# AIS-Bonn/lattice_net

Hardware: AMD Instinct MI355X
Metric: Mpoints/sec splat+conv+slice fwd+bwd on 120k-pt SemanticKITTI scan (higher is better)
Workload: dtype f32 (convolution products bf16x3-emulated)

## Files before the change

### include/latticenet_hip.h

```cpp
#ifndef LATTICENET_HIP_H
#define LATTICENET_HIP_H

#include <stddef.h>

#ifdef __cplusplus
extern "C" {
#endif

#define LN_OK 0
#define LN_ERR_ARG (-1)
#define LN_ERR_UNSUPPORTED (-2)
#define LN_ERR_LAUNCH (-3)
#define LN_ERR_WORKSPACE (-4)

#define LN_STATUS_TABLE_FULL 1
#define LN_STATUS_KEY_RANGE 2
#define LN_STATUS_BUCKET_OVERFLOW 4

#define LN_MAX_POS_DIM 6
#define LN_SLOT_MAP_INTS 32
#define LN_KEYS_RAW 0
#define LN_KEYS_LATTICE 1
#define LN_NOT_VISITED (-2)

// ... 44 lines not shown

int ln_table_bucket_count(int capacity);
int ln_build_concurrency(int scans_in_flight);

size_t ln_build_workspace_bytes(long long tokens, int capacity);

#define LN_BUILD_WRITE_IDX 1
#define LN_BUILD_CLEAR_FIRST 2
#define LN_BUILD_ATOMIC_PATH 4
#define LN_BUILD_CANONICAL_ROWS 8
#define LN_BUILD_SORTED_CSR 16
int ln_build_splat(const LnTable* t, const float* positions_raw, const float* sigmas_host, int n, int* idx, float* w,
                   int flags, const LnCsr* csr, void* workspace, size_t workspace_bytes, float* clear_values,
                   long long clear_values_elems, void* stream);

int ln_canonicalize(const LnTable* t, int* idx, long long tokens, const LnCsr* csr, void* workspace, size_t workspace_bytes, void* stream);

int ln_rehash(const LnTable* t, void* stream);

int ln_splat_accumulate(float* table_values, const float* vals, const int* idx, const float* w, int n, int pos_dim,
                        int val_dim, void* stream);

long long ln_csr_max_segments(long long tokens, int groups_upper);
size_t ln_csr_workspace_bytes(long long tokens, int groups_upper);
int ln_csr_build(const int* idx, long long tokens, int groups_upper, const LnCsr* csr, void* workspace, size_t workspace_bytes,
                 void* stream);
int ln_csr_reduce_rows(const LnCsr* csr, const int* grp_row, long long max_segments, const float* src, const float* w, int val_dim,
                       int src_div, int src_stride, float* dst, void* stream);
int ln_csr_sort(const LnCsr* csr, int groups_upper, void* workspace, size_t workspace_bytes, long long tokens, void* stream);

// ... 144 lines not shown
```

### lattice_net_amd/_lib.py

```python
from __future__ import annotations

import ctypes as C
import os

import torch

_PKG = os.path.dirname(os.path.abspath(__file__))
LIB_PATH = os.environ.get("LATTICE_NET_LIB") or os.path.join(_PKG, "liblatticenet_hip.so")

LN_STATUS_TABLE_FULL = 1
LN_STATUS_KEY_RANGE = 2
LN_STATUS_BUCKET_OVERFLOW = 4
LN_BUILD_WRITE_IDX = 1
LN_BUILD_CLEAR_FIRST = 2
LN_BUILD_ATOMIC_PATH = 4
LN_BUILD_CANONICAL_ROWS = 8
LN_BUILD_SORTED_CSR = 16
LN_NOT_VISITED = -2
LN_CONV_FLIP_NEIGHBOURS = 1
LN_CONV_TRANSPOSED_FILTER = 2
LN_CONV_BANK_READY = 4
LN_MAX_POS_DIM = 6
LN_KEYS_RAW = 0
LN_KEYS_LATTICE = 1
LN_XCD_GROUPS = 8
LN_SLOT_MAP_INTS = 32


class LnTable(C.Structure):

    _fields_ = [
        ("capacity", C.c_int),
# ... 39 lines not shown
_CSR = C.POINTER(LnCsr)

SIGNATURES = {
    "ln_last_error_string": (C.c_char_p, []),
    "ln_version": (C.c_char_p, []),
    "ln_abi_hash": (C.c_char_p, []),
    "ln_kernel_names": (C.c_char_p, []),
    "ln_profile_begin": (_i, [C.c_char_p, _i]),
    "ln_profile_end": (_i, [C.POINTER(C.c_double), C.POINTER(_i)]),
    "ln_profile_end_table": (_i, [C.c_char_p, _i]),
    "ln_table_clear": (_i, [_T, _vp, _ll, _vp]),
    "ln_build_workspace_bytes": (_sz, [_ll, _i]),
    "ln_table_bucket_count": (_i, [_i]),
    "ln_build_concurrency": (_i, [_i]),
    "ln_build_splat": (_i, [_T, _vp, _vp, _i, _vp, _vp, _i, _CSR, _vp, _sz, _vp, _ll, _vp]),
    "ln_rehash": (_i, [_T, _vp]),
    "ln_canonicalize": (_i, [_T, _vp, _ll, _CSR, _vp, _sz, _vp]),
    "ln_splat_accumulate": (_i, [_vp, _vp, _vp, _vp, _i, _i, _i, _vp]),
    "ln_csr_workspace_bytes": (_sz, [_ll, _i]),
    "ln_csr_max_segments": (_ll, [_ll, _i]),
    "ln_csr_build": (_i, [_vp, _ll, _i, _CSR, _vp, _sz, _vp]),
    "ln_csr_reduce_rows": (_i, [_CSR, _vp, _ll, _vp, _vp, _i, _i, _i, _vp, _vp]),
    "ln_csr_sort": (_i, [_CSR, _i, _vp, _sz, _ll, _vp]),
    "ln_splat_accumulate_and_neighbours": (_i, [_CSR, _vp, _ll, _vp, _vp, _i, _i, _i, _vp, _T, _i, _vp, _vp]),
    "ln_csr_segment_max": (_i, [_CSR, _vp, _ll, _vp, _i, _i, _vp, _vp, _vp, _vp]),
    "ln_csr_group_sizes": (_i, [_CSR, _vp, _i, _i, _vp, _vp]),
    "ln_distribute": (_i, [_T, _vp, _vp, _vp, _i, _i, _vp, _vp, _vp, _i, _CSR, _vp, _sz, _vp, _ll, _vp]),
    "ln_coarsen": (_i, [_T, _i, _T, _CSR, _vp, _sz, _vp]),
    "ln_neighbours": (_i, [_T, _i, _T, _i, _i, _i, _i, _vp, _vp]),
    "ln_im2row": (_i, [_vp, _vp, _i, _i, _i, _vp, _vp]),
# ... 108 lines not shown
```

### lattice_net_amd/csrc/ln_table.hip

```cpp
#include "ln_common.h"
#include "ln_simplex.h"
#include "ln_csr.h"
#include "ln_neighbours.h"

#include <stdarg.h>
#include <stdio.h>
#include <string.h>

static thread_local char g_ln_error[512] = "";

void ln_set_error(const char* fmt, ...) {
    va_list ap;
    va_start(ap, fmt);
    vsnprintf(g_ln_error, sizeof(g_ln_error), fmt, ap);
    va_end(ap);
}

int ln_check_launch(const char* what) {
    hipError_t e = hipGetLastError();
    if (e != hipSuccess) {
        ln_set_error("%s: %s", what, hipGetErrorString(e));
        return LN_ERR_LAUNCH;
    }
    return LN_OK;
}

extern "C" const char* ln_last_error_string(void) { return g_ln_error; }

#include <vector>
namespace {
struct LnProfState {
    char names[256] = "";
    int max_samples = 0;
    std::vector<hipEvent_t> starts, stops;
    std::vector<const char*> sample_names;
    size_t used = 0;
    long long dropped = 0;
};
LnProfState g_prof;
}

LnProfEvents ln_prof_next(const char* name) {
    LnProfEvents ev{nullptr, nullptr, false};
// ... 283 lines not shown
        for (int i = 0; i < D; ++i) o[i] = pr[i] / sc.sigma[i];
        for (int j = 0; j < val_dim; ++j) o[D + j] = vals[(size_t)p * val_dim + j];
        o[D + val_dim] = b;
    }
}


#ifndef LN_KEYS_PTS_SMALL_D
#define LN_KEYS_PTS_SMALL_D 2
#endif
#define LN_KEYS_PTS_PER_THREAD ((D) <= 3 ? LN_KEYS_PTS_SMALL_D : 1)
#define LN_KEYS_PTS_PER_BLOCK (256 * LN_KEYS_PTS_PER_THREAD)
template <int D, int TH>
__global__ void __launch_bounds__(TH)
    k_point_keys(LnTable t, const float* __restrict__ pos_raw, LnScale<D> sc, int n, int sb, int nbk, int capb,
                 int* __restrict__ part_tok, unsigned long long* __restrict__ part_pk, int* __restrict__ tok_slot,
                 float* __restrict__ w, const float* __restrict__ vals, int val_dim, float* __restrict__ distributed,
                 int* __restrict__ seg_count, int seg_regions, float* __restrict__ clear_values, long long clear_values_elems,
                 unsigned int* __restrict__ pub) {
    constexpr bool SPLIT = TH == 1024;
    constexpr int PTS = TH == 256 ? LN_KEYS_PTS_PER_THREAD : 1;
    constexpr int RH = SPLIT ? (D + 2) / 2 : D + 1;
    constexpr int PTS_PER_BLOCK = SPLIT ? 512 : TH * PTS;
    __shared__ int s_cnt[LN_BKT_MAX];
    __shared__ int s_lbase[LN_BKT_MAX];
    __shared__ int s_scan_tmp[TH / 64];
    __shared__ unsigned long long s_stage_pk[PTS_PER_BLOCK * (D + 1)];
    __shared__ int s_stage_tok[PTS_PER_BLOCK * (D + 1)];
    __shared__ int s_stage_dst[PTS_PER_BLOCK * (D + 1)];
    int* cursor = t.slot_cnt;
    LN_STAMP(0);
    for (int b = threadIdx.x; b < nbk; b += TH) s_cnt[b] = 0;
    const LnSlotMap smap = ln_load_slot_map(t.slot_map);
    ln_lds_barrier();
    LN_STAMP(1);
    unsigned long long pk[PTS][RH];
    int bkt[PTS][RH];
    int rank[PTS][RH];
    bool bad_key = false;
    const int r_first = SPLIT ? (threadIdx.x & 1) * RH : 0;
#pragma unroll
    for (int it = 0; it < PTS; ++it) {
        const int p = SPLIT ? blockIdx.x * PTS_PER_BLOCK + (threadIdx.x >> 1) : blockIdx.x * PTS_PER_BLOCK + it * TH + threadIdx.x;
#pragma unroll
        for (int k = 0; k < RH; ++k) bkt[it][k] = -1;
        if (p >= n) continue;
        float pr[D];
#pragma unroll
        for (int i = 0; i < D; ++i) pr[i] = pos_raw[(size_t)p * D + i];
        LnSimplex<D> s;
        ln_simplex<D>(pr, sc, s);
        ln_simplex_of_cloud<D>(s, p, t.batch_points, t.batch_key_step);
#pragma unroll
        for (int k = 0; k < RH; ++k) {
            const int r = r_first + k;
            if (SPLIT && r > D) continue;
            int key[D];
            ln_vertex_key<D>(s, r, key);
            float bary = s.bary[0];
#pragma unroll
            for (int q = 1; q <= D; ++q) bary = (r == q) ? s.bary[q] : bary;
            const size_t tk = (size_t)p * (D + 1) + r;
            const bool lat_fmt = t.key_format == LN_KEYS_LATTICE;
            const bool ok = lat_fmt ? KeyPack<D>::lattice_in_range(key, r) : KeyPack<D>::in_range(key, t.key_format);
            if (ok) {
                pk[it][k] = lat_fmt ? KeyPack<D>::lattice_pack(key, r) : KeyPack<D>::pack(key, t.key_format);
                bkt[it][k] = LnProbe::bucket_of_key<D>(key, t.capacity, sb, smap);
                rank[it][k] = atomicAdd(&s_cnt[bkt[it][k]], 1);
            } else {
                bad_key = true;
                if (tok_slot) tok_slot[tk] = -1;
            }
            if (w) w[tk] = ok ? bary : -1.0f;
            if (distributed) {
                const int row_len = D + val_dim + 1;
                float* o = distributed + tk * row_len;
#pragma unroll
// ... 22 lines not shown
    }
    LN_STAMP(4);
    ln_lds_barrier();
    LN_STAMP(5);
#pragma unroll
    for (int it = 0; it < PTS; ++it) {
        const int p = SPLIT ? blockIdx.x * PTS_PER_BLOCK + (threadIdx.x >> 1) : blockIdx.x * PTS_PER_BLOCK + it * TH + threadIdx.x;
#pragma unroll
        for (int k = 0; k < RH; ++k) {
            if (bkt[it][k] < 0) continue;
            const int tk = p * (D + 1) + r_first + k;
            const int at = s_cnt[bkt[it][k]] + rank[it][k];
            const int j = s_lbase[bkt[it][k]] + rank[it][k];
            s_stage_tok[j] = tk;
            s_stage_pk[j] = pk[it][k];
            s_stage_dst[j] = at < capb ? bkt[it][k] * capb + at : -1;
        }
    }
    ln_lds_barrier();
    LN_STAMP(6);
    for (int j = threadIdx.x; j < block_tokens; j += TH) {
        const int dst = s_stage_dst[j];
        const int tk = s_stage_tok[j];
        if (dst >= 0) {
            part_tok[dst] = tk;
            part_pk[dst] = s_stage_pk[j];
        } else if (tok_slot) {
            tok_slot[tk] = -1;
        }
    }
    {
        const long long stride = (long long)gridDim.x * TH;
        const long long g = (long long)blockIdx.x * TH + threadIdx.x;
        if (clear_values) {
            const long long n4 = clear_values_elems >> 2;
            float4* v4 = reinterpret_cast<float4*>(clear_values);
            for (long long i = g; i < n4; i += stride) v4[i] = make_float4(0.f, 0.f, 0.f, 0.f);
            for (long long i = (n4 << 2) + g; i < clear_values_elems; i += stride) clear_values[i] = 0.f;
        }
        const long long nk = (long long)t.capacity * D;
        for (long long i = g; i < nk; i += stride) t.keys[i] = 0;
// ... 12 lines not shown
#ifndef LN_BKT_THREADS
#define LN_BKT_THREADS 1024
#endif
#define LN_BKT_WAVES (LN_BKT_THREADS / 64)
#ifndef LN_BKT_NARROW_TOKENS
#define LN_BKT_NARROW_TOKENS 4096
#endif
static thread_local int g_ln_build_concurrency = 1;
extern "C" int ln_build_concurrency(int scans_in_flight) {
    g_ln_build_concurrency = scans_in_flight > 1 ? scans_in_flight : 1;
    return LN_OK;
}
#define LN_BKT_LDS_LIMIT (150 * 1024)
#define LN_BKT_LDS_PER_SLOT (sizeof(unsigned long long) + 7 * sizeof(int))
#define LN_BKT_LDS_EXTRA 32
#ifndef LN_BKT_REG_TOK
#define LN_BKT_REG_TOK 4
#endif
#define LN_PUB_READY 0x80000000u
#define LN_PUB_ERR 0x40000000u
#define LN_PUB_CNT 0x3FFFFFFFu
template <int D, int TH>
__global__ void __launch_bounds__(TH)
    k_bucket_rows(LnTable t, int sb, int nbk, int capb, int* __restrict__ cursor, const int* __restrict__ part_tok,
                  const unsigned long long* __restrict__ part_pk, int* __restrict__ part_slot, int* __restrict__ part_pos,
                  int* __restrict__ idx_out, LnCsr csr, unsigned int* __restrict__ pub) {
    extern __shared__ __attribute__((aligned(16))) unsigned long long s_mem[];
    unsigned long long* skeys = s_mem;
    int* scnt = reinterpret_cast<int*>(skeys + sb);
    unsigned int* smin = reinterpret_cast<unsigned int*>(scnt + sb);
    int* soff = reinterpret_cast<int*>(smin + sb);
    int* sseg = soff + sb;
    int* srow = sseg + sb;
    int* srank = srow + sb;
    unsigned int* slist = reinterpret_cast<unsigned int*>(s_mem) + ((8 * sb + 3) & ~3);
    __shared__ int s_wave_tok[16], s_wave_seg[16], s_wave_new[16];
    __shared__ int s_run_tok, s_run_seg, s_run_new, s_err;
    __shared__ int s_rcnt[LN_XCD_GROUPS], s_rbase[LN_XCD_GROUPS];
    __shared__ int s_ticket;
    const int tid = threadIdx.x;
    const int lane = tid & 63;
    const int wave = tid >> 6;
    if (tid == 0) s_ticket = atomicAdd(reinterpret_cast<int*>(&pub[nbk]), 1);
    LN_STAMP(8);
    for (int i = tid; i < sb; i += TH) {
        skeys[i] = LN_EMPTY_KEY;
        scnt[i] = 0;
        smin[i] = LN_EMPTY_TOK;
    }
    ln_lds_barrier();
    const int b = s_ticket;
    const bool mapped = t.slot_map != nullptr;
    const LnBucket bk(b, t.capacity, sb, t.slot_map);
    const int lo = bk.lo;
    const int size = bk.size;
    const size_t in0 = (size_t)b * capb;
    int before = 0;
    for (int i = tid; i < b; i += TH) before += min(cursor[i], capb);
    const int my_cursor = cursor[b];
    const int ntok = min(my_cursor, capb);
    int r_tk[LN_BKT_REG_TOK], r_ls[LN_BKT_REG_TOK], r_pos[LN_BKT_REG_TOK];
    unsigned long long r_pk[LN_BKT_REG_TOK];
#pragma unroll
    for (int k = 0; k < LN_BKT_REG_TOK; ++k) {
        const int j = tid + k * TH;
        r_ls[k] = -1;
        r_pos[k] = -1;
        r_tk[k] = j < ntok ? part_tok[in0 + j] : -1;
        r_pk[k] = j < ntok ? part_pk[in0 + j] : LN_EMPTY_KEY;
    }
#pragma unroll
    for (int off = 32; off >= 1; off >>= 1) before += __shfl_xor(before, off, 64);
    if (lane == 0) s_wave_tok[wave] = before;
    if (tid == 0) {
        s_run_tok = 0;
        s_run_seg = 0;
        s_run_new = 0;
        s_err = my_cursor > capb ? 1 : 0;
    }
    if (tid < LN_XCD_GROUPS) s_rcnt[tid] = 0;
    __syncthreads();
    int base = 0;
#pragma unroll
    for (int k = 0; k < (TH / 64); ++k) base += s_wave_tok[k];
// ... 191 lines not shown
    const int new_here = s_run_new;
    if (t.row_regions && tid == 0 && slot_ordered) {
        const int bpr = nbk / LN_XCD_GROUPS;
        if (b % bpr == 0) t.row_regions[b / bpr] = base_row;
        if (b == nbk - 1) t.row_regions[LN_XCD_GROUPS] = base_row + new_here;
    }
    LN_STAMP(12);
    for (int i = tid; i < size; i += TH) {
        const int h = lo + i;
        const int beg = base + soff[i];
        const int c = scnt[i];
        int row = -1;
        if (c) {
            row = base_row + srow[i];
            if (t.row_limit > 0 && row >= t.row_limit) row = -1;
        }
        srow[i] = row;
        csr.grp_start[h] = beg;
        const unsigned long long pk = skeys[i];
        t.slot_keys[h] = pk;
        t.entries[h] = row;
        t.slot_tok[h] = smin[i];
        if (row >= 0) {
            int key[D];
            KeyPack<D>::unpack(pk, key, t.key_format);
#pragma unroll
            for (int k = 0; k < D; ++k) t.keys[(size_t)row * D + k] = key[k];
        }
        const int sr = planes ? (sseg[i] >> 28) : bucket_region;
        long long sid = (long long)sr * csr.seg_region + s_rbase[planes ? sr : 0] + (planes ? (sseg[i] & 0x0FFFFFFF) : sseg[i]);
// ... 8 lines not shown
            t.slot_tok[h] = LN_EMPTY_TOK;
        }
        if (tid == 0) {
            csr.grp_start[t.capacity] = base + ntok;
            const int total = base_row + new_here;
            int bits = (err_all ? LN_STATUS_BUCKET_OVERFLOW : 0) | (cursor[nbk] ? LN_STATUS_KEY_RANGE : 0);
            *t.nr_filled = total;
            if (bits) atomicOr(t.status, bits);
            ln_report_to_host(t.host_counters, total, bits, t.host_seq);
        }
        __syncthreads();
        for (int i = tid; i <= nbk; i += TH) cursor[i] = 0;
    }
    ln_lds_barrier();
    LN_STAMP(13);
#pragma unroll
    for (int k = 0; k < LN_BKT_REG_TOK; ++k) {
        if (r_tk[k] < 0) continue;
        if (r_ls[k] >= 0) csr.csr_tok[base + soff[r_ls[k]] + r_pos[k]] = r_tk[k];
        if (idx_out) idx_out[r_tk[k]] = r_ls[k] >= 0 ? srow[r_ls[k]] : -1;
    }
    for (int j = tid + LN_BKT_REG_TOK * TH; j < ntok; j += TH) {
        const int ls = part_slot[in0 + j];
        const int tk = part_tok[in0 + j];
        if (ls >= 0) csr.csr_tok[base + soff[ls] + part_pos[in0 + j]] = tk;
        if (idx_out) idx_out[tk] = ls >= 0 ? srow[ls] : -1;
    }
    for (int j = placed + tid; j < ntok; j += TH)
        csr.csr_tok[base + j] = -1;
    LN_STAMP(14);
}

template <int D>
__global__ void __launch_bounds__(256)
    k_insert_coarse(LnTable fine, int fine_rows_upper, LnTable coarse, int* __restrict__ tok_slot, int* __restrict__ tok_pos) {
    constexpr int TPR = 2 * (D + 1) + 1;
    const int r = blockIdx.x * blockDim.x + threadIdx.x;
    int m = *fine.nr_filled;
    if (m > fine_rows_upper) m = fine_rows_upper;
    if (r >= fine_rows_upper) return;
    int* ts = tok_slot + (size_t)r * TPR;
    int* tp = tok_pos + (size_t)r * TPR;
    for (int j = 0; j < TPR; ++j) {
        ts[j] = -1;
        tp[j] = -1;
// ... 168 lines not shown

struct BuildWs {
    unsigned long long* bitmap;
    int* block_cnt;
    int* block_prefix;
    int* tok_slot;
    int* tok_pos;
    void* csr_ws;
    size_t csr_ws_bytes;
    int nb;
    int capb;
    unsigned long long* part_pk;
    int* part_tok;
    int* part_slot;
    int* part_pos;
    unsigned int* pub;
};

static size_t ln_align256(size_t x) { return (x + 255) & ~size_t(255); }

static int ln_bucket_region(long long tokens, int capacity) {
    const int nbk = ln_bucket_count(capacity);
    long long capb = 16 * ((tokens + nbk - 1) / nbk) + 1024;
    capb = (capb + 63) & ~63ll;
    return int(capb);
}

extern "C" int ln_table_bucket_count(int capacity) { return capacity > 0 ? ln_bucket_count(capacity) : 0; }

extern "C" size_t ln_build_workspace_bytes(long long tokens, int capacity) {
    if (tokens < 1) tokens = 1;
    if (capacity < 1) capacity = 1;
    const size_t nb = (size_t)ln_div_up(tokens, 256);
    const size_t region = (size_t)ln_bucket_count(capacity) * ln_bucket_region(tokens, capacity);
    return ln_align256(nb * 4 * sizeof(unsigned long long)) + 2 * ln_align256(nb * sizeof(int)) +
           2 * ln_align256((size_t)tokens * sizeof(int)) + ln_align256(ln_csr_scan_workspace_bytes(capacity)) +
           ln_align256(region * sizeof(unsigned long long)) + 3 * ln_align256(region * sizeof(int)) +
           ln_align256(((size_t)ln_bucket_count(capacity) + 1) * sizeof(unsigned int));
}

static int ln_carve_ws(long long tokens, int capacity, void* workspace, size_t bytes, BuildWs& ws) {
    LN_REQUIRE(workspace != nullptr && bytes >= ln_build_workspace_bytes(tokens, capacity), LN_ERR_WORKSPACE,
               "build workspace too small: %zu < %zu", bytes, ln_build_workspace_bytes(tokens, capacity));
    LN_REQUIRE((reinterpret_cast<uintptr_t>(workspace) & 255) == 0, LN_ERR_WORKSPACE, "build workspace must be 256-byte aligned");
    LN_REQUIRE(tokens < 0x7FFFFFFFll, LN_ERR_ARG, "too many insertion tokens: %lld", tokens);
    char* p = static_cast<char*>(workspace);
    ws.nb = ln_div_up(tokens, 256);
    ws.bitmap = reinterpret_cast<unsigned long long*>(p);
    p += ln_align256((size_t)ws.nb * 4 * sizeof(unsigned long long));
    ws.block_cnt = reinterpret_cast<int*>(p);
    p += ln_align256((size_t)ws.nb * sizeof(int));
    ws.block_prefix = reinterpret_cast<int*>(p);
// ... 3 lines not shown
    ws.tok_pos = reinterpret_cast<int*>(p);
    p += ln_align256((size_t)tokens * sizeof(int));
    ws.csr_ws = p;
    ws.csr_ws_bytes = ln_csr_scan_workspace_bytes(capacity);
    p += ln_align256(ws.csr_ws_bytes);
    ws.capb = ln_bucket_region(tokens, capacity);
    const size_t region = (size_t)ln_bucket_count(capacity) * ws.capb;
    ws.part_pk = reinterpret_cast<unsigned long long*>(p);
    p += ln_align256(region * sizeof(unsigned long long));
    ws.part_tok = reinterpret_cast<int*>(p);
    p += ln_align256(region * sizeof(int));
    ws.part_slot = reinterpret_cast<int*>(p);
    p += ln_align256(region * sizeof(int));
    ws.part_pos = reinterpret_cast<int*>(p);
    p += ln_align256(region * sizeof(int));
    ws.pub = reinterpret_cast<unsigned int*>(p);
    return LN_OK;
}

template <int D>
static int ln_rank_rows(const LnTable& t, const int* tok_slot, int* idx_out, long long tokens, const BuildWs& ws, hipStream_t st);

template <int D>
static int ln_rank_and_finalize(const LnTable& t, const int* tok_slot, const int* tok_pos, int* idx_out, long long tokens,
                                const BuildWs& ws, const LnCsr& csr, hipStream_t st) {
    int rc = ln_csr_from_counts(tok_slot, tok_pos, tokens, t.slot_cnt, t.capacity, csr, ws.csr_ws, ws.csr_ws_bytes, st);
    if (rc) return rc;
    const long long max_seg = ln_csr_max_segments(tokens, t.capacity);
    LN_LAUNCH("k_seg_min", k_seg_min, dim3(ln_div_up(max_seg, 256)), dim3(256), 0, st, t, csr.csr_tok,
              reinterpret_cast<const int4*>(csr.seg_desc), csr.seg_count);
// ... 57 lines not shown
    LN_LAUNCH("k_scan_blocks", k_scan_blocks, dim3(1), dim3(1024), 0, st, (const int*)nullptr, ws.bitmap, ws.nb, ws.block_prefix, t.nr_filled, t.status,
              (int*)nullptr, 0, 1);
    LN_LAUNCH("k_canon_slots", k_canon_slots<D>, dim3(slot_blocks), dim3(256), 0, st, t, ws.bitmap, ws.block_prefix, ws.tok_pos);
    if (idx) LN_LAUNCH("k_canon_idx", k_canon_idx, dim3(ws.nb), dim3(256), 0, st, idx, tokens, ws.tok_pos);
    if (csr && csr->seg_desc && csr->seg_count)
        LN_LAUNCH("k_canon_segs", k_canon_segs, dim3(ln_div_up((long long)LN_XCD_GROUPS * csr->seg_region, 256)), dim3(256), 0, st,
                  reinterpret_cast<int4*>(csr->seg_desc), csr->seg_count, csr->seg_region, ws.tok_pos);
    return ln_check_launch("ln_canonicalize");
}

static int ln_check_csr(const LnCsr* c, const char* who) {
    LN_REQUIRE(c && c->grp_start && c->csr_tok && c->seg_desc && (reinterpret_cast<uintptr_t>(c->seg_desc) & 15) == 0 && c->seg_count, LN_ERR_ARG, "%s: CSR output has a null buffer", who);
    return LN_OK;
}

static int ln_build_points(const LnTable* t, const float* positions_raw, const float* sigmas_host, int n, int* idx, float* w,
                           int flags, const float* vals, int val_dim, float* distributed, const LnCsr* csr, void* workspace,
                           size_t workspace_bytes, float* clear_values, long long clear_values_elems, void* stream, const char* who) {
    int rc = ln_check_table(t, who);
    if (rc) return rc;
    rc = ln_check_csr(csr, who);
    if (rc) return rc;
    const int write_idx = flags & LN_BUILD_WRITE_IDX;
    LN_REQUIRE(n >= 0, LN_ERR_ARG, "%s: n=%d", who, n);
    LN_REQUIRE(positions_raw != nullptr || n == 0, LN_ERR_ARG, "%s: null positions", who);
    LN_REQUIRE(!write_idx || n == 0 || (idx && w), LN_ERR_ARG, "%s: write_idx set but idx/w null", who);
    const long long tokens = (long long)n * (t->pos_dim + 1);
    BuildWs ws;
    if (n > 0) {
        rc = ln_carve_ws(tokens, t->capacity, workspace, workspace_bytes, ws);
        if (rc) return rc;
    }
    const int sb_lds = (t->slot_map && t->bucket_slots_max > 0) ? t->bucket_slots_max : ln_bucket_slots(t->capacity);
// ... 4 lines not shown
    LN_REQUIRE(clear_values == nullptr || (reinterpret_cast<uintptr_t>(clear_values) & 15) == 0, LN_ERR_ARG, "%s: clear_values must be 16-byte aligned", who);
    if ((flags & LN_BUILD_CLEAR_FIRST) && !bucketed) {
        rc = ln_table_clear(t, clear_values, clear_values_elems, stream);
        if (rc) return rc;
    }
    if (n == 0) return LN_OK;
    hipStream_t st = (hipStream_t)stream;
    int* tok_slot = write_idx ? idx : ws.tok_slot;
    LN_DISPATCH_D(t->pos_dim, {
        LnScale<D> sc = ln_make_scale<D>(sigmas_host);
        if (bucketed) {
            const int sb = sb_lds;
            const int nbk = t->slot_map ? (ln_bucket_count(t->capacity) / LN_XCD_GROUPS) * LN_XCD_GROUPS : ln_bucket_count(t->capacity);
            const size_t lds = bucket_lds;
            int* dropped_idx = write_idx ? idx : (int*)nullptr;
            if (D <= 3)
                LN_LAUNCH("k_point_keys", (k_point_keys<D, (D <= 3 ? 512 : 256)>), dim3(ln_div_up(n, 512)), dim3(512), 0, st, *t, positions_raw, sc, n, sb,
                          nbk, ws.capb, ws.part_tok, ws.part_pk, dropped_idx, write_idx ? w : (float*)nullptr, vals, val_dim, distributed,
                          csr->seg_count, csr->planes ? LN_XCD_GROUPS : 1, clear_values, clear_values_elems, ws.pub);
            else
                LN_LAUNCH("k_point_keys", (k_point_keys<D, 256>), dim3(ln_div_up(n, LN_KEYS_PTS_PER_BLOCK)), dim3(256), 0, st, *t, positions_raw, sc, n, sb,
                          nbk, ws.capb, ws.part_tok, ws.part_pk, dropped_idx, write_idx ? w : (float*)nullptr, vals, val_dim, distributed,
                          csr->seg_count, csr->planes ? LN_XCD_GROUPS : 1, clear_values, clear_values_elems, ws.pub);
            const bool narrow = g_ln_build_concurrency > 1 && tokens <= (long long)LN_BKT_NARROW_TOKENS * nbk;
            if (narrow)
                LN_LAUNCH("k_bucket_rows", (k_bucket_rows<D, 512>), dim3(nbk), dim3(512), lds, st, *t, sb, nbk, ws.capb, t->slot_cnt,
                      ws.part_tok, ws.part_pk, ws.part_slot, ws.part_pos, dropped_idx, *csr, ws.pub);
            else
                LN_LAUNCH("k_bucket_rows", (k_bucket_rows<D, LN_BKT_THREADS>), dim3(nbk), dim3(LN_BKT_THREADS), lds, st, *t, sb, nbk, ws.capb, t->slot_cnt,
                      ws.part_tok, ws.part_pk, ws.part_slot, ws.part_pos, dropped_idx, *csr, ws.pub);
            rc = ln_check_launch(who);
            if (rc == LN_OK && (flags & LN_BUILD_CANONICAL_ROWS)) rc = ln_canonicalize_impl<D>(*t, dropped_idx, tokens, csr, ws, st);
            if (rc == LN_OK && (flags & LN_BUILD_SORTED_CSR)) rc = ln_csr_sort_groups(*csr, t->capacity, ws.tok_slot, st);
        } else {
            LN_LAUNCH("k_insert_points", k_insert_points<D>, dim3(ln_div_up(tokens, 256)), dim3(256), 0, st, *t, positions_raw, sc, n, tok_slot,
                      ws.tok_pos, write_idx ? w : (float*)nullptr, vals, val_dim, distributed);
            rc = ln_rank_and_finalize<D>(*t, tok_slot, ws.tok_pos, write_idx ? idx : (int*)nullptr, tokens, ws, *csr, st);
            if (rc == LN_OK && (flags & LN_BUILD_SORTED_CSR)) rc = ln_csr_sort_groups(*csr, t->capacity, ws.tok_pos, st);
        }
    });
    return rc;
}

extern "C" int ln_build_splat(const LnTable* t, const float* positions_raw, const float* sigmas_host, int n, int* idx,
                              float* w, int flags, const LnCsr* csr, void* workspace, size_t workspace_bytes, float* clear_values,
                              long long clear_values_elems, void* stream) {
    return ln_build_points(t, positions_raw, sigmas_host, n, idx, w, flags, nullptr, 0, nullptr, csr, workspace, workspace_bytes,
                           clear_values, clear_values_elems, stream, "ln_build_splat");
}

extern "C" int ln_distribute(const LnTable* t, const float* positions_raw, const float* sigmas_host, const float* vals, int n,
                             int val_dim, int* idx, float* w, float* distributed, int flags, const LnCsr* csr, void* workspace,
                             size_t workspace_bytes, float* clear_values, long long clear_values_elems, void* stream) {
    LN_REQUIRE(vals && distributed && idx && w, LN_ERR_ARG, "ln_distribute: null buffer");
    LN_REQUIRE(val_dim >= 1, LN_ERR_ARG, "ln_distribute: val_dim=%d", val_dim);
    return ln_build_points(t, positions_raw, sigmas_host, n, idx, w, flags | LN_BUILD_WRITE_IDX, vals, val_dim, distributed, csr, workspace,
                           workspace_bytes, clear_values, clear_values_elems, stream, "ln_distribute");
}

__global__ void __launch_bounds__(256) k_rehash_clear(LnTable t) {
    const long long stride = (long long)gridDim.x * 256;
    for (long long i = (long long)blockIdx.x * 256 + threadIdx.x; i < t.capacity; i += stride) {
        t.slot_keys[i] = LN_EMPTY_KEY;
// ... 140 lines not shown
```

### lattice_net_amd/lattice.py

```python
from __future__ import annotations

import ctypes as C
import itertools
import os
import re
import weakref
from typing import Optional, Sequence

import torch
import torch.utils.weak

from . import _lib

__all__ = ["Lattice", "HashTable", "set_row_order", "get_row_order", "set_hash_capacity_policy", "set_slot_order", "set_bank_cache", "set_deterministic"]


_SIZE_CACHE = {}
_FORCE_ATOMIC_BUILD = os.environ.get("LATTICE_BUILD_PATH", "") == "atomic"

_ROW_ORDER = [os.environ.get("LATTICE_ROW_ORDER", "slot")]


_HASH_POLICY = [os.environ.get("LATTICE_HASH_CAPACITY", "tokens")]
_STATIC_SLOTS_PER_ROW = float(os.environ.get("LATTICE_STATIC_SLOTS_PER_ROW", "2.3"))
# ... 31 lines not shown
    _PLANES_KEEPALIVE.append(t)
    return t, int(sb.max())
_ORDERED_SLICE = [os.environ.get("LATTICE_ORDERED_SLICE", "0") == "1"]


def set_slot_order(order: str) -> str:
    if order not in ("space", "hash"):
        raise ValueError(f"slot order must be 'space' or 'hash', got {order!r}")
    prev, _SLOT_ORDER[0] = _SLOT_ORDER[0], order
    return prev


_SCANS_IN_FLIGHT = [max(1, int(os.environ.get("LATTICE_SCANS_IN_FLIGHT", "1")))]


def set_scans_in_flight(n: int) -> int:
    prev, _SCANS_IN_FLIGHT[0] = _SCANS_IN_FLIGHT[0], max(1, int(n))
    return prev


_DETERMINISTIC = [os.environ.get("LATTICE_DETERMINISTIC", "0") == "1"]


def set_deterministic(on: bool) -> bool:
    prev, _DETERMINISTIC[0] = _DETERMINISTIC[0], bool(on)
    return prev


def set_hash_capacity_policy(policy: str) -> str:
    if policy not in ("tokens", "full"):
# ... 90 lines not shown
        arena = torch.empty((kw + ew + cw + 4 + sw,), dtype=torch.int32, device=device)
        _lib.check(_lib.load().ln_arena_init(_lib.ptr(arena), arena.numel(), kw, kw + capacity, _lib.stream_ptr(arena.device)), "ln_arena_init")
        self.keys = arena[: capacity * pos_dim].view(capacity, pos_dim)
        self.entries = arena[kw: kw + capacity]
        self.slot_cnt = arena[kw + ew: kw + ew + capacity]
        self.fresh_counters = arena[kw + ew + cw: kw + ew + cw + 2]
        if spare_row_width > 0:
            self.fresh_row = arena[kw + ew + cw + 4: kw + ew + cw + 4 + spare_row_width].view(torch.float32).view(1, spare_row_width)
        self.slot_keys = torch.empty((capacity,), dtype=torch.int64, device=device)
        self.slot_tok = torch.empty((capacity,), dtype=torch.int32, device=device)
        self.key_format = _lib.LN_KEYS_LATTICE
        self.version = 0
        self.nbr_cache = {}
        self.csr_cache = {}
        self.replay = None
        self.planes = None
        self.plane_values = None
        self.leaf_shares = None
        self.slot_map = None
        self.slot_map_sb_max = 0
        self.row_regions = None
        self.rows_follow_space = False

    def adopt_planes(self):
        self.rows_follow_space = False
        if self.planes is None or _SLOT_ORDER[0] != "space":
            self.slot_map, self.slot_map_sb_max = None, 0
            return
        key = (self.plane_values, self.leaf_shares, self.hashed())
        hit = _SLOT_MAPS.get(key)
# ... 334 lines not shown
        if not self.m_hash_table.is_initialized():
            self.m_hash_table.init(pos_dim, val_dim, self._dev(like))

    def _alloc_csr(self, tokens: int, groups_upper: int, planes=None):
        max_seg = _build_sizes(tokens, groups_upper)[2]
        tk = max(tokens, 1)
        G = _lib.LN_XCD_GROUPS
        buf = torch.empty((4 * G * max_seg + groups_upper + 1 + tk + G + 2,), dtype=torch.int32, device=self._dev())
        base = buf.data_ptr()
        o1 = 4 * G * max_seg
        o2 = o1 + groups_upper + 1
        o3 = o2 + tk
        c = _lib.LnCsr(base + 4 * o1, base + 4 * o2, base, base + 4 * o3, max_seg, _lib.ptr(planes))
        return buf, c, max_seg

    def _build(self, positions_raw, write: bool, vals=None, distributed=None):
        n, d = positions_raw.shape
        dev = self._dev(positions_raw)
        ht = self.m_hash_table
        idx = w = None
        if write:
            idx = torch.empty((n * (d + 1),), dtype=torch.int32, device=dev)
            w = torch.empty((n * (d + 1),), dtype=torch.float32, device=dev)
        tokens = n * (d + 1)
        st = ht._storage
        clear_vals, do_clear = ht.take_pending_clear()
        self._choose_hash_capacity(tokens, fresh=do_clear)
        if do_clear:
            st.adopt_planes()
        cap = st.hashed()
        csr_buf, csr, max_seg = self._alloc_csr(tokens, cap, st.planes)
# ... 10 lines not shown
            lib = _lib.load()
            if force_atomic and st.slot_map is not None:
                st.slot_map, st.slot_map_sb_max = None, 0
            ws = self._workspace(_build_sizes(tokens, cap)[0])
            t = ht.c_table()
            flags = (_lib.LN_BUILD_WRITE_IDX if write else 0) | (_lib.LN_BUILD_CLEAR_FIRST if do_clear else 0)
            if force_atomic or _FORCE_ATOMIC_BUILD:
                flags |= _lib.LN_BUILD_ATOMIC_PATH
            if _ROW_ORDER[0] == "canonical":
                flags |= _lib.LN_BUILD_CANONICAL_ROWS
            if _DETERMINISTIC[0]:
                flags |= _lib.LN_BUILD_SORTED_CSR
            cv, cn = _lib.ptr(clear_vals), clear_elems
            lib.ln_build_concurrency(_SCANS_IN_FLIGHT[0])
            ht.arm_count_readback()
            if distributed is None:
                rc = lib.ln_build_splat(C.byref(t), _lib.ptr(positions_raw), self._sigmas_host(), n, _lib.ptr(idx), _lib.ptr(w), flags,
                                        C.byref(csr), _lib.ptr(ws), ws.numel(), cv, cn, self._stream())
                _lib.check(rc, "ln_build_splat")
            else:
                rc = lib.ln_distribute(C.byref(t), _lib.ptr(positions_raw), self._sigmas_host(), _lib.ptr(vals), n, vals.shape[1],
                                       _lib.ptr(idx), _lib.ptr(w), _lib.ptr(distributed), flags, C.byref(csr), _lib.ptr(ws), ws.numel(),
                                       cv, cn, self._stream())
                _lib.check(rc, "ln_distribute")
            st.touch()
            st.rows_follow_space = bool(st.slot_map is not None and do_clear and not (flags & (_lib.LN_BUILD_ATOMIC_PATH | _lib.LN_BUILD_CANONICAL_ROWS)))
            ht.m_nr_filled_is_dirty = True
            if n > 0 and ht._static_rows is None:
                ht.start_count_readback()
            else:
                ht._readback_pending = False
# ... 127 lines not shown
        cap = ht._static_rows if ht._static_rows is not None else ht.capacity()
        if tv is None or tuple(tv.shape) != (cap, v) or tv.requires_grad or tv._base is not None or not tv.is_contiguous():
            pending = getattr(ht, "_clear_pending", False)
            ht._clear_pending = False
            if pending:
                self._choose_hash_capacity(n * (d + 1), fresh=True)
                reach = min(cap, ht._storage.hashed())
                ht.m_values_tensor = torch.empty((cap, v), dtype=torch.float32, device=self._dev(positions_raw))
                if reach < cap:
                    ht.m_values_tensor[reach:].zero_()
                ht._zero_beyond = (weakref.ref(ht.m_values_tensor), reach)
            else:
                ht.m_values_tensor = torch.zeros((cap, v), dtype=torch.float32, device=self._dev(positions_raw))
                ht._zero_beyond = (weakref.ref(ht.m_values_tensor), 0)
            ht._clear_pending = pending
        idx, w = self._build(positions_raw, True)
        tv = ht.m_values_tensor
        self._after_build(lambda: self._accumulate_and_prefetch(values, idx, w, tv, v, d + 1, n * (d + 1)))
        self._trace_level()
        return idx, w

    def just_create_verts(self, positions_raw: torch.Tensor, return_indices_and_weights: bool):
        self._check_positions(positions_raw)
        d = positions_raw.shape[1]
        self._ensure_table(d, 1, positions_raw)
        idx, w = self._build(positions_raw, bool(return_indices_and_weights))
        self._trace_level()
        return idx, w

    def distribute(self, positions_raw: torch.Tensor, values: torch.Tensor, reset_hashmap: bool = True):
        self._check_positions_and_values(positions_raw, values)
        n, d = positions_raw.shape
# ... 36 lines not shown
        oh, nh = self.m_hash_table, new.m_hash_table
        nh._storage = oh._storage.clone()
        nh.m_values_tensor = torch.zeros((1, self.val_dim()), dtype=torch.float32, device=self._dev())
        nh._counters = oh._counters.clone()
        new.just_create_verts(pos.contiguous(), False)
        if expand_values:
            diff = new.nr_lattice_vertices() - self.nr_lattice_vertices()
            if diff < 0:
                raise _lib.LatticeNetHipError("expand produced fewer vertices than the source lattice")
            new.set_values(torch.nn.functional.pad(self.values()[: self.nr_lattice_vertices()], (0, 0, 0, diff)))
        return new

    def _accumulate_and_prefetch(self, values, idx, w, dst, val_dim, src_div, tokens):
        ht = self.m_hash_table
        st = ht._storage
        rows_upper = min(ht.capacity(), tokens)
        _, csr, max_seg, grp_row, _ = self._csr(idx)
        if rows_upper <= 0 or max_seg <= 0 or not self.prefetch_neighbours:
            return self._scatter_rows(values, idx, w, dst, val_dim, src_div, val_dim)
        lib = _lib.load()
        nbr = torch.empty((rows_upper, self.get_filter_extent(1)), dtype=torch.int32, device=self._dev())
        t = ht.c_table()
        fn, what = (lib.ln_splat_accumulate_and_neighbours_f16, "ln_splat_accumulate_and_neighbours_f16") if values.dtype == torch.float16 \
            else (lib.ln_splat_accumulate_and_neighbours, "ln_splat_accumulate_and_neighbours")
        csr.dense = self._dense_hint(tokens)
        _lib.check(fn(C.byref(csr), _lib.ptr(grp_row), max_seg, _lib.ptr(values), _lib.ptr(w), val_dim, src_div, val_dim, _lib.ptr(dst),
                      C.byref(t), rows_upper, _lib.ptr(nbr), self._stream()), what)
        st.nbr_cache[("prefetch", st.uid, st.version, self.m_lvl)] = (nbr,)

    def _prefetch_neighbours(self, tokens: int):
# ... 670 lines not shown
```

Measured before the change: 1466.

## Fuse splat value accumulation into bucket-row hash build kernel

Carries the barycentric weights through the key-partition stage (new part_w workspace) and lets k_bucket_rows accumulate the weighted value rows directly into the lattice values tensor. It stages token offset and weight pairs in LDS when they fit, and falls back to reading the CSR from global memory otherwise. Heavy segments are split across a wavefront. The goal is to drop the separate accumulate kernel and its CSR re-read. The trade-off is higher LDS use and more registers in the build kernel, which may lower occupancy. Neighbour prefetch then runs as its own pass, where before it was fused with accumulation.

```diff
diff --git a/include/latticenet_hip.h b/include/latticenet_hip.h
--- a/include/latticenet_hip.h
+++ b/include/latticenet_hip.h
@@ -82,6 +82,11 @@
                    int flags, const LnCsr* csr, void* workspace, size_t workspace_bytes, float* clear_values,
                    long long clear_values_elems, void* stream);
 
+#define LN_BUILD_NOT_ACCUMULATED 1
+int ln_build_splat_accumulate(const LnTable* t, const float* positions_raw, const float* sigmas_host, int n, int* idx, float* w,
+                              int flags, const LnCsr* csr, void* workspace, size_t workspace_bytes, float* clear_values,
+                              long long clear_values_elems, const float* vals, int val_dim, float* values, void* stream);
+
 int ln_canonicalize(const LnTable* t, int* idx, long long tokens, const LnCsr* csr, void* workspace, size_t workspace_bytes, void* stream);
 
 int ln_rehash(const LnTable* t, void* stream);
diff --git a/lattice_net_amd/_lib.py b/lattice_net_amd/_lib.py
--- a/lattice_net_amd/_lib.py
+++ b/lattice_net_amd/_lib.py
@@ -16,6 +16,7 @@
 LN_BUILD_ATOMIC_PATH = 4
 LN_BUILD_CANONICAL_ROWS = 8
 LN_BUILD_SORTED_CSR = 16
+LN_BUILD_NOT_ACCUMULATED = 1
 LN_NOT_VISITED = -2
 LN_CONV_FLIP_NEIGHBOURS = 1
 LN_CONV_TRANSPOSED_FILTER = 2
@@ -85,6 +86,7 @@
     "ln_table_bucket_count": (_i, [_i]),
     "ln_build_concurrency": (_i, [_i]),
     "ln_build_splat": (_i, [_T, _vp, _vp, _i, _vp, _vp, _i, _CSR, _vp, _sz, _vp, _ll, _vp]),
+    "ln_build_splat_accumulate": (_i, [_T, _vp, _vp, _i, _vp, _vp, _i, _CSR, _vp, _sz, _vp, _ll, _vp, _i, _vp, _vp]),
     "ln_rehash": (_i, [_T, _vp]),
     "ln_canonicalize": (_i, [_T, _vp, _ll, _CSR, _vp, _sz, _vp]),
     "ln_splat_accumulate": (_i, [_vp, _vp, _vp, _vp, _i, _i, _i, _vp]),
diff --git a/lattice_net_amd/csrc/ln_table.hip b/lattice_net_amd/csrc/ln_table.hip
--- a/lattice_net_amd/csrc/ln_table.hip
+++ b/lattice_net_amd/csrc/ln_table.hip
@@ -27,6 +27,8 @@
 
 extern "C" const char* ln_last_error_string(void) { return g_ln_error; }
 
+#include <algorithm>
+#include <type_traits>
 #include <vector>
 namespace {
 struct LnProfState {
@@ -340,8 +342,8 @@
 template <int D, int TH>
 __global__ void __launch_bounds__(TH)
     k_point_keys(LnTable t, const float* __restrict__ pos_raw, LnScale<D> sc, int n, int sb, int nbk, int capb,
-                 int* __restrict__ part_tok, unsigned long long* __restrict__ part_pk, int* __restrict__ tok_slot,
-                 float* __restrict__ w, const float* __restrict__ vals, int val_dim, float* __restrict__ distributed,
+                 int* __restrict__ part_tok, unsigned long long* __restrict__ part_pk, float* __restrict__ part_w,
+                 int* __restrict__ tok_slot, float* __restrict__ w, const float* __restrict__ vals, int val_dim, float* __restrict__ distributed,
                  int* __restrict__ seg_count, int seg_regions, float* __restrict__ clear_values, long long clear_values_elems,
                  unsigned int* __restrict__ pub) {
     constexpr bool SPLIT = TH == 1024;
@@ -354,6 +356,7 @@
     __shared__ unsigned long long s_stage_pk[PTS_PER_BLOCK * (D + 1)];
     __shared__ int s_stage_tok[PTS_PER_BLOCK * (D + 1)];
     __shared__ int s_stage_dst[PTS_PER_BLOCK * (D + 1)];
+    __shared__ float s_stage_w[PTS_PER_BLOCK * (D + 1)];
     int* cursor = t.slot_cnt;
     LN_STAMP(0);
     for (int b = threadIdx.x; b < nbk; b += TH) s_cnt[b] = 0;
@@ -363,6 +366,7 @@
     unsigned long long pk[PTS][RH];
     int bkt[PTS][RH];
     int rank[PTS][RH];
+    float bw[PTS][RH];
     bool bad_key = false;
     const int r_first = SPLIT ? (threadIdx.x & 1) * RH : 0;
 #pragma unroll
@@ -387,6 +391,7 @@
 #pragma unroll
             for (int q = 1; q <= D; ++q) bary = (r == q) ? s.bary[q] : bary;
             const size_t tk = (size_t)p * (D + 1) + r;
+            bw[it][k] = bary;
             const bool lat_fmt = t.key_format == LN_KEYS_LATTICE;
             const bool ok = lat_fmt ? KeyPack<D>::lattice_in_range(key, r) : KeyPack<D>::in_range(key, t.key_format);
             if (ok) {
@@ -439,6 +444,7 @@
             const int j = s_lbase[bkt[it][k]] + rank[it][k];
             s_stage_tok[j] = tk;
             s_stage_pk[j] = pk[it][k];
+            s_stage_w[j] = bw[it][k];
             s_stage_dst[j] = at < capb ? bkt[it][k] * capb + at : -1;
         }
     }
@@ -450,6 +456,7 @@
         if (dst >= 0) {
             part_tok[dst] = tk;
             part_pk[dst] = s_stage_pk[j];
+            if (part_w) part_w[dst] = s_stage_w[j];
         } else if (tok_slot) {
             tok_slot[tk] = -1;
         }
@@ -492,17 +499,73 @@
 #define LN_BKT_LDS_LIMIT (150 * 1024)
 #define LN_BKT_LDS_PER_SLOT (sizeof(unsigned long long) + 7 * sizeof(int))
 #define LN_BKT_LDS_EXTRA 32
+#define LN_BKT_STAGE_OFFSET(sb) ((9 * (sb) + 8 + 1) / 2)
 #ifndef LN_BKT_REG_TOK
 #define LN_BKT_REG_TOK 4
 #endif
 #define LN_PUB_READY 0x80000000u
 #define LN_PUB_ERR 0x40000000u
 #define LN_PUB_CNT 0x3FFFFFFFu
-template <int D, int TH>
+struct LnBucketAcc {
+    const float* part_w;
+    const float* vals;
+    const float* w;
+    float* values;
+    int val_dim;
+    int stage_cap;
+};
+
+template <bool STAGED, bool SAFE, int D>
+__device__ __forceinline__ float4 ln_bucket_unit_sum(const int2* __restrict__ stage, const int* __restrict__ csr_tok, const float* __restrict__ w,
+                                                     const float* __restrict__ vals, int val_dim, int beg, int end, int lane_off) {
+    float4 acc = make_float4(0.f, 0.f, 0.f, 0.f);
+    for (int e0 = beg; e0 < end; e0 += 4) {
+        int2 en[4];
+#pragma unroll
+        for (int u = 0; u < 4; ++u) {
+            const int e = min(e0 + u, end - 1);
+            if constexpr (STAGED) {
+                en[u] = stage[e];
+            } else {
+                const int tk = max(__hip_atomic_load(&csr_tok[e], __ATOMIC_RELAXED, __HIP_MEMORY_SCOPE_AGENT), 0);
+                en[u] = make_int2((tk / (D + 1)) * val_dim, __float_as_int(w[tk]));
+            }
+        }
+        float4 x[4];
+        float wt[4];
+#pragma unroll
+        for (int u = 0; u < 4; ++u) {
+            const bool valid = e0 + u < end;
+            wt[u] = valid ? __int_as_float(en[u].y) : 0.f;
+            x[u] = *reinterpret_cast<const float4*>(vals + (unsigned int)(en[u].x + lane_off));
+            if constexpr (SAFE)
+                if (!valid) x[u] = make_float4(0.f, 0.f, 0.f, 0.f);
+        }
+#pragma unroll
+        for (int u = 0; u < 4; ++u) {
+            acc.x = fmaf(x[u].x, wt[u], acc.x);
+            acc.y = fmaf(x[u].y, wt[u], acc.y);
+            acc.z = fmaf(x[u].z, wt[u], acc.z);
+            acc.w = fmaf(x[u].w, wt[u], acc.w);
+        }
+    }
+    return acc;
+}
+
+template <bool STAGED, int D>
+__device__ __forceinline__ float4 ln_bucket_unit(const int2* __restrict__ stage, const int* __restrict__ csr_tok, const float* __restrict__ w,
+                                                 const float* __restrict__ vals, int val_dim, int beg, int end, int lane_off) {
+    float4 a = ln_bucket_unit_sum<STAGED, false, D>(stage, csr_tok, w, vals, val_dim, beg, end, lane_off);
+    if (a.x != a.x || a.y != a.y || a.z != a.z || a.w != a.w)
+        a = ln_bucket_unit_sum<STAGED, true, D>(stage, csr_tok, w, vals, val_dim, beg, end, lane_off);
+    return a;
+}
+
+template <int D, int TH, int ACC = 0>
 __global__ void __launch_bounds__(TH)
     k_bucket_rows(LnTable t, int sb, int nbk, int capb, int* __restrict__ cursor, const int* __restrict__ part_tok,
                   const unsigned long long* __restrict__ part_pk, int* __restrict__ part_slot, int* __restrict__ part_pos,
-                  int* __restrict__ idx_out, LnCsr csr, unsigned int* __restrict__ pub) {
+                  int* __restrict__ idx_out, LnCsr csr, unsigned int* __restrict__ pub, LnBucketAcc ac) {
     extern __shared__ __attribute__((aligned(16))) unsigned long long s_mem[];
     unsigned long long* skeys = s_mem;
     int* scnt = reinterpret_cast<int*>(skeys + sb);
@@ -512,6 +575,7 @@
     int* srow = sseg + sb;
     int* srank = srow + sb;
     unsigned int* slist = reinterpret_cast<unsigned int*>(s_mem) + ((8 * sb + 3) & ~3);
+    int2* stage = reinterpret_cast<int2*>(s_mem) + LN_BKT_STAGE_OFFSET(sb);
     __shared__ int s_wave_tok[16], s_wave_seg[16], s_wave_new[16];
     __shared__ int s_run_tok, s_run_seg, s_run_new, s_err;
     __shared__ int s_rcnt[LN_XCD_GROUPS], s_rbase[LN_XCD_GROUPS];
@@ -539,6 +603,7 @@
     const int ntok = min(my_cursor, capb);
     int r_tk[LN_BKT_REG_TOK], r_ls[LN_BKT_REG_TOK], r_pos[LN_BKT_REG_TOK];
     unsigned long long r_pk[LN_BKT_REG_TOK];
+    float r_w[LN_BKT_REG_TOK];
 #pragma unroll
     for (int k = 0; k < LN_BKT_REG_TOK; ++k) {
         const int j = tid + k * TH;
@@ -546,6 +611,7 @@
         r_pos[k] = -1;
         r_tk[k] = j < ntok ? part_tok[in0 + j] : -1;
         r_pk[k] = j < ntok ? part_pk[in0 + j] : LN_EMPTY_KEY;
+        if constexpr (ACC != 0) r_w[k] = j < ntok ? ac.part_w[in0 + j] : 0.f;
     }
 #pragma unroll
     for (int off = 32; off >= 1; off >>= 1) before += __shfl_xor(before, off, 64);
@@ -767,6 +833,7 @@
         if (c) {
             row = base_row + srow[i];
             if (t.row_limit > 0 && row >= t.row_limit) row = -1;
+            if constexpr (ACC != 0) slist[srow[i]] = (unsigned int)i;
         }
         srow[i] = row;
         csr.grp_start[h] = beg;
@@ -805,21 +872,97 @@
     }
     ln_lds_barrier();
     LN_STAMP(13);
+    const bool staged = ntok <= ac.stage_cap;
 #pragma unroll
     for (int k = 0; k < LN_BKT_REG_TOK; ++k) {
         if (r_tk[k] < 0) continue;
-        if (r_ls[k] >= 0) csr.csr_tok[base + soff[r_ls[k]] + r_pos[k]] = r_tk[k];
+        if (r_ls[k] >= 0) {
+            const int p = soff[r_ls[k]] + r_pos[k];
+            csr.csr_tok[base + p] = r_tk[k];
+            if constexpr (ACC != 0)
+                if (staged) stage[p] = make_int2((r_tk[k] / (D + 1)) * ac.val_dim, __float_as_int(r_w[k]));
+        }
         if (idx_out) idx_out[r_tk[k]] = r_ls[k] >= 0 ? srow[r_ls[k]] : -1;
     }
     for (int j = tid + LN_BKT_REG_TOK * TH; j < ntok; j += TH) {
         const int ls = part_slot[in0 + j];
         const int tk = part_tok[in0 + j];
-        if (ls >= 0) csr.csr_tok[base + soff[ls] + part_pos[in0 + j]] = tk;
+        if (ls >= 0) {
+            const int p = soff[ls] + part_pos[in0 + j];
+            csr.csr_tok[base + p] = tk;
+            if constexpr (ACC != 0)
+                if (staged) stage[p] = make_int2((tk / (D + 1)) * ac.val_dim, __float_as_int(ac.part_w[in0 + j]));
+        }
         if (idx_out) idx_out[tk] = ls >= 0 ? srow[ls] : -1;
     }
     for (int j = placed + tid; j < ntok; j += TH)
         csr.csr_tok[base + j] = -1;
     LN_STAMP(14);
+    if constexpr (ACC != 0) {
+        if (staged) {
+            ln_lds_barrier();
+        } else {
+            __threadfence();
+            __syncthreads();
+        }
+        const int chunks = ac.val_dim >> 2;
+        int lps = ACC == 8 ? 8 : 1;
+        if constexpr (ACC != 8)
+            while (lps < chunks) lps <<= 1;
+        const int lps_shift = __ffs(lps) - 1;
+        const int gpw = 64 >> lps_shift;
+        const int lc = lane & (lps - 1), g = lane >> lps_shift;
+        const bool cok = lc < chunks;
+        const int lane_off = cok ? lc * 4 : 0;
+        const int* __restrict__ ctok = csr.csr_tok + base;
+        auto walk = [&](auto staged_c) {
+            constexpr bool ST = decltype(staged_c)::value;
+            for (int v0 = wave * gpw; v0 < new_here; v0 += (TH / 64) * gpw) {
+                const int v = v0 + g;
+                int c = 0, off = 0, row = -1;
+                if (v < new_here) {
+                    const int i = (int)slist[v];
+                    c = scnt[i];
+                    off = soff[i];
+                    row = srow[i];
+                }
+                if (row >= 0 && c <= LN_CSR_SEG && cok) {
+                    const float4 a = ln_bucket_unit<ST, D>(stage, ctok, ac.w, ac.vals, ac.val_dim, off, off + c, lane_off);
+                    *reinterpret_cast<float4*>(ac.values + (size_t)row * ac.val_dim + lane_off) = a;
+                }
+                unsigned long long hot = __ballot(row >= 0 && c > LN_CSR_SEG && lc == 0);
+                while (hot) {
+                    const int src = __ffsll((long long)hot) - 1;
+                    hot &= hot - 1;
+                    const int h_c = __shfl(c, src, 64), h_off = __shfl(off, src, 64), h_row = __shfl(row, src, 64);
+                    float4 a = make_float4(0.f, 0.f, 0.f, 0.f);
+                    const int ulen = min(LN_CSR_SEG, (((h_c + gpw - 1) >> (6 - lps_shift)) + 3) & ~3);
+                    if (cok) {
+                        for (int e = g * ulen; e < h_c; e += gpw * ulen) {
+                            const float4 u = ln_bucket_unit<ST, D>(stage, ctok, ac.w, ac.vals, ac.val_dim, h_off + e,
+                                                                   h_off + min(h_c, e + ulen), lane_off);
+                            a.x += u.x;
+                            a.y += u.y;
+                            a.z += u.z;
+                            a.w += u.w;
+                        }
+                    }
+                    for (int o = lps; o < 64; o <<= 1) {
+                        a.x += __shfl_xor(a.x, o, 64);
+                        a.y += __shfl_xor(a.y, o, 64);
+                        a.z += __shfl_xor(a.z, o, 64);
+                        a.w += __shfl_xor(a.w, o, 64);
+                    }
+                    if (g == 0 && cok) *reinterpret_cast<float4*>(ac.values + (size_t)h_row * ac.val_dim + lane_off) = a;
+                }
+            }
+        };
+        if (staged)
+            walk(std::true_type{});
+        else
+            walk(std::false_type{});
+        LN_STAMP(18);
+    }
 }
 
 template <int D>
@@ -1018,6 +1161,7 @@
     int* part_tok;
     int* part_slot;
     int* part_pos;
+    float* part_w;
     unsigned int* pub;
 };
 
@@ -1039,7 +1183,7 @@
     const size_t region = (size_t)ln_bucket_count(capacity) * ln_bucket_region(tokens, capacity);
     return ln_align256(nb * 4 * sizeof(unsigned long long)) + 2 * ln_align256(nb * sizeof(int)) +
            2 * ln_align256((size_t)tokens * sizeof(int)) + ln_align256(ln_csr_scan_workspace_bytes(capacity)) +
-           ln_align256(region * sizeof(unsigned long long)) + 3 * ln_align256(region * sizeof(int)) +
+           ln_align256(region * sizeof(unsigned long long)) + 3 * ln_align256(region * sizeof(int)) + ln_align256(region * sizeof(float)) +
            ln_align256(((size_t)ln_bucket_count(capacity) + 1) * sizeof(unsigned int));
 }
 
@@ -1073,6 +1217,8 @@
     p += ln_align256(region * sizeof(int));
     ws.part_pos = reinterpret_cast<int*>(p);
     p += ln_align256(region * sizeof(int));
+    ws.part_w = reinterpret_cast<float*>(p);
+    p += ln_align256(region * sizeof(float));
     ws.pub = reinterpret_cast<unsigned int*>(p);
     return LN_OK;
 }
@@ -1160,9 +1306,14 @@
     return LN_OK;
 }
 
+#define LN_BUCKET_LAUNCH(THREADS, ACCV, LDSB)                                                                                          \
+    LN_LAUNCH("k_bucket_rows", (k_bucket_rows<D, THREADS, ACCV>), dim3(nbk), dim3(THREADS), LDSB, st, *t, sb, nbk, ws.capb, t->slot_cnt, \
+              ws.part_tok, ws.part_pk, ws.part_slot, ws.part_pos, dropped_idx, *csr, ws.pub, ac)
 static int ln_build_points(const LnTable* t, const float* positions_raw, const float* sigmas_host, int n, int* idx, float* w,
                            int flags, const float* vals, int val_dim, float* distributed, const LnCsr* csr, void* workspace,
-                           size_t workspace_bytes, float* clear_values, long long clear_values_elems, void* stream, const char* who) {
+                           size_t workspace_bytes, float* clear_values, long long clear_values_elems, void* stream, const char* who,
+                           const float* acc_vals = nullptr, int acc_val_dim = 0, float* acc_values = nullptr, bool* accumulated = nullptr) {
+    if (accumulated) *accumulated = false;
     int rc = ln_check_table(t, who);
     if (rc) return rc;
     rc = ln_check_csr(csr, who);
@@ -1197,22 +1348,39 @@
             const int nbk = t->slot_map ? (ln_bucket_count(t->capacity) / LN_XCD_GROUPS) * LN_XCD_GROUPS : ln_bucket_count(t->capacity);
             const size_t lds = bucket_lds;
             int* dropped_idx = write_idx ? idx : (int*)nullptr;
+            LnBucketAcc ac{};
+            size_t lds_acc = 0;
+            if (acc_vals && acc_values && write_idx && !(flags & (LN_BUILD_CANONICAL_ROWS | LN_BUILD_SORTED_CSR)) && acc_val_dim >= 4 &&
+                acc_val_dim % 4 == 0 && acc_val_dim <= 64 && (long long)n * acc_val_dim < 0x7FFFFFFFll &&
+                ((reinterpret_cast<uintptr_t>(acc_vals) | reinterpret_cast<uintptr_t>(acc_values)) & 15) == 0) {
+                long long cap = 2 * ((tokens + nbk - 1) / nbk) + 512;
+                cap = std::min<long long>((cap + 63) & ~63ll, ws.capb);
+                lds_acc = ((size_t)LN_BKT_STAGE_OFFSET(sb) + (size_t)cap) * sizeof(int2);
+                if (lds_acc <= LN_BKT_LDS_LIMIT) ac = LnBucketAcc{ws.part_w, acc_vals, w, acc_values, acc_val_dim, int(cap)};
+            }
+            const bool acc = ac.vals != nullptr;
+            float* part_w = acc ? ws.part_w : (float*)nullptr;
             if (D <= 3)
                 LN_LAUNCH("k_point_keys", (k_point_keys<D, (D <= 3 ? 512 : 256)>), dim3(ln_div_up(n, 512)), dim3(512), 0, st, *t, positions_raw, sc, n, sb,
-                          nbk, ws.capb, ws.part_tok, ws.part_pk, dropped_idx, write_idx ? w : (float*)nullptr, vals, val_dim, distributed,
+                          nbk, ws.capb, ws.part_tok, ws.part_pk, part_w, dropped_idx, write_idx ? w : (float*)nullptr, vals, val_dim, distributed,
                           csr->seg_count, csr->planes ? LN_XCD_GROUPS : 1, clear_values, clear_values_elems, ws.pub);
             else
                 LN_LAUNCH("k_point_keys", (k_point_keys<D, 256>), dim3(ln_div_up(n, LN_KEYS_PTS_PER_BLOCK)), dim3(256), 0, st, *t, positions_raw, sc, n, sb,
-                          nbk, ws.capb, ws.part_tok, ws.part_pk, dropped_idx, write_idx ? w : (float*)nullptr, vals, val_dim, distributed,
+                          nbk, ws.capb, ws.part_tok, ws.part_pk, part_w, dropped_idx, write_idx ? w : (float*)nullptr, vals, val_dim, distributed,
                           csr->seg_count, csr->planes ? LN_XCD_GROUPS : 1, clear_values, clear_values_elems, ws.pub);
             const bool narrow = g_ln_build_concurrency > 1 && tokens <= (long long)LN_BKT_NARROW_TOKENS * nbk;
-            if (narrow)
-                LN_LAUNCH("k_bucket_rows", (k_bucket_rows<D, 512>), dim3(nbk), dim3(512), lds, st, *t, sb, nbk, ws.capb, t->slot_cnt,
-                      ws.part_tok, ws.part_pk, ws.part_slot, ws.part_pos, dropped_idx, *csr, ws.pub);
-            else
-                LN_LAUNCH("k_bucket_rows", (k_bucket_rows<D, LN_BKT_THREADS>), dim3(nbk), dim3(LN_BKT_THREADS), lds, st, *t, sb, nbk, ws.capb, t->slot_cnt,
-                      ws.part_tok, ws.part_pk, ws.part_slot, ws.part_pos, dropped_idx, *csr, ws.pub);
+            if (acc && acc_val_dim == 32) {
+                if (narrow) LN_BUCKET_LAUNCH(512, 8, lds_acc);
+                else LN_BUCKET_LAUNCH(LN_BKT_THREADS, 8, lds_acc);
+            } else if (acc) {
+                if (narrow) LN_BUCKET_LAUNCH(512, 1, lds_acc);
+                else LN_BUCKET_LAUNCH(LN_BKT_THREADS, 1, lds_acc);
+            } else {
+                if (narrow) LN_BUCKET_LAUNCH(512, 0, lds);
+                else LN_BUCKET_LAUNCH(LN_BKT_THREADS, 0, lds);
+            }
             rc = ln_check_launch(who);
+            if (rc == LN_OK && acc && accumulated) *accumulated = true;
             if (rc == LN_OK && (flags & LN_BUILD_CANONICAL_ROWS)) rc = ln_canonicalize_impl<D>(*t, dropped_idx, tokens, csr, ws, st);
             if (rc == LN_OK && (flags & LN_BUILD_SORTED_CSR)) rc = ln_csr_sort_groups(*csr, t->capacity, ws.tok_slot, st);
         } else {
@@ -1230,6 +1398,18 @@
                               long long clear_values_elems, void* stream) {
     return ln_build_points(t, positions_raw, sigmas_host, n, idx, w, flags, nullptr, 0, nullptr, csr, workspace, workspace_bytes,
                            clear_values, clear_values_elems, stream, "ln_build_splat");
+}
+
+extern "C" int ln_build_splat_accumulate(const LnTable* t, const float* positions_raw, const float* sigmas_host, int n, int* idx,
+                                         float* w, int flags, const LnCsr* csr, void* workspace, size_t workspace_bytes,
+                                         float* clear_values, long long clear_values_elems, const float* vals, int val_dim,
+                                         float* values, void* stream) {
+    LN_REQUIRE(val_dim >= 1 && (n == 0 || (vals && values)), LN_ERR_ARG, "ln_build_splat_accumulate: null rows / val_dim=%d", val_dim);
+    bool accumulated = false;
+    const int rc = ln_build_points(t, positions_raw, sigmas_host, n, idx, w, flags, nullptr, 0, nullptr, csr, workspace, workspace_bytes,
+                                   clear_values, clear_values_elems, stream, "ln_build_splat_accumulate", vals, val_dim, values, &accumulated);
+    if (rc != LN_OK) return rc;
+    return accumulated ? LN_OK : LN_BUILD_NOT_ACCUMULATED;
 }
 
 extern "C" int ln_distribute(const LnTable* t, const float* positions_raw, const float* sigmas_host, const float* vals, int n,
diff --git a/lattice_net_amd/lattice.py b/lattice_net_amd/lattice.py
--- a/lattice_net_amd/lattice.py
+++ b/lattice_net_amd/lattice.py
@@ -69,6 +69,15 @@
 _SCANS_IN_FLIGHT = [max(1, int(os.environ.get("LATTICE_SCANS_IN_FLIGHT", "1")))]
 
 
+_ACCUMULATE_IN_BUILD = [True, True]
+
+
+def set_accumulate_in_build(alone: bool, in_flight: bool):
+    prev = tuple(_ACCUMULATE_IN_BUILD)
+    _ACCUMULATE_IN_BUILD[:] = [bool(alone), bool(in_flight)]
+    return prev
+
+
 def set_scans_in_flight(n: int) -> int:
     prev, _SCANS_IN_FLIGHT[0] = _SCANS_IN_FLIGHT[0], max(1, int(n))
     return prev
@@ -189,6 +198,7 @@
         self.nbr_cache = {}
         self.csr_cache = {}
         self.replay = None
+        self.accumulated_in_build = False
         self.planes = None
         self.plane_values = None
         self.leaf_shares = None
@@ -553,7 +563,7 @@
         c = _lib.LnCsr(base + 4 * o1, base + 4 * o2, base, base + 4 * o3, max_seg, _lib.ptr(planes))
         return buf, c, max_seg
 
-    def _build(self, positions_raw, write: bool, vals=None, distributed=None):
+    def _build(self, positions_raw, write: bool, vals=None, distributed=None, accumulate=None):
         n, d = positions_raw.shape
         dev = self._dev(positions_raw)
         ht = self.m_hash_table
@@ -594,7 +604,18 @@
             cv, cn = _lib.ptr(clear_vals), clear_elems
             lib.ln_build_concurrency(_SCANS_IN_FLIGHT[0])
             ht.arm_count_readback()
-            if distributed is None:
+            st.accumulated_in_build = False
+            if distributed is None and accumulate is not None and write and not force_atomic and _ACCUMULATE_IN_BUILD[1 if _SCANS_IN_FLIGHT[0] > 1 else 0]:
+                src, dst = accumulate
+                rc = lib.ln_build_splat_accumulate(C.byref(t), _lib.ptr(positions_raw), self._sigmas_host(), n, _lib.ptr(idx), _lib.ptr(w),
+                                                   flags, C.byref(csr), _lib.ptr(ws), ws.numel(), cv, cn, _lib.ptr(src), int(src.shape[1]),
+                                                   _lib.ptr(dst), self._stream())
+                if rc != _lib.LN_BUILD_NOT_ACCUMULATED:
+                    _lib.check(rc, "ln_build_splat_accumulate")
+                    st.accumulated_in_build = True
+            elif distributed is None:
+                if force_atomic and accumulate is not None and cv is None:
+                    accumulate[1].zero_()
                 rc = lib.ln_build_splat(C.byref(t), _lib.ptr(positions_raw), self._sigmas_host(), n, _lib.ptr(idx), _lib.ptr(w), flags,
                                         C.byref(csr), _lib.ptr(ws), ws.numel(), cv, cn, self._stream())
                 _lib.check(rc, "ln_build_splat")
@@ -752,8 +773,8 @@
                 ht.m_values_tensor = torch.zeros((cap, v), dtype=torch.float32, device=self._dev(positions_raw))
                 ht._zero_beyond = (weakref.ref(ht.m_values_tensor), 0)
             ht._clear_pending = pending
-        idx, w = self._build(positions_raw, True)
         tv = ht.m_values_tensor
+        idx, w = self._build(positions_raw, True, accumulate=(values, tv) if values.dtype == torch.float32 else None)
         self._after_build(lambda: self._accumulate_and_prefetch(values, idx, w, tv, v, d + 1, n * (d + 1)))
         self._trace_level()
         return idx, w
@@ -820,6 +841,10 @@
     def _accumulate_and_prefetch(self, values, idx, w, dst, val_dim, src_div, tokens):
         ht = self.m_hash_table
         st = ht._storage
+        if getattr(st, "accumulated_in_build", False):
+            if self.prefetch_neighbours:
+                self._prefetch_neighbours(tokens)
+            return
         rows_upper = min(ht.capacity(), tokens)
         _, csr, max_seg, grp_row, _ = self._csr(idx)
         if rows_upper <= 0 or max_seg <= 0 or not self.prefetch_neighbours:
```

Result: slower. 1448 (-1.2%).
